# NIRVANALAN/LN3Diff

Hardware: NVIDIA H100
Metric: denoised-latents/sec (higher is better)
Workload: dtype bf16

## Files before the change

### ln3diff_b200/csrc/attention_wgmma.cu

```cuda
#include <cstdlib>

#include "common.cuh"
#include "ln3_internal.h"

namespace ln3 {

static constexpr int kQT = 128;
static constexpr int kKT = 128;
static constexpr int kHD = 64;
static constexpr int kTileBytes = 128 * kHD * 2;
static constexpr int kStages = 4;
static constexpr int kThreads = 2 * 128 + 32;
static constexpr int kFmhaSmem = 1024 + kTileBytes * (1 + 2 * kStages) + 256;

struct FmhaParams {
  int Lq, Lkv, Lkv2;
  int nb1, nb2;
  float scale_log2;
  int causal;
  __nv_bfloat16* out;
  long long o_ld, o_bs;
};

__global__ void __launch_bounds__(kThreads, 1)
fmha_fwd_kernel(const __grid_constant__ CUtensorMap tmap_q, const __grid_constant__ CUtensorMap tmap_k,
                const __grid_constant__ CUtensorMap tmap_v, const __grid_constant__ CUtensorMap tmap_k2,
                const __grid_constant__ CUtensorMap tmap_v2, const FmhaParams p) {
  extern __shared__ uint8_t smem_raw[];
  uint8_t* smem = reinterpret_cast<uint8_t*>((reinterpret_cast<uintptr_t>(smem_raw) + 1023) &
                                             ~static_cast<uintptr_t>(1023));
  uint8_t* sQ = smem;
  uint8_t* sK = sQ + kTileBytes;
  uint8_t* sV = sK + kStages * kTileBytes;
  uint64_t* bars = reinterpret_cast<uint64_t*>(sV + kStages * kTileBytes);
  uint64_t* q_full = bars;
  uint64_t* kv_full = bars + 1;
  uint64_t* kv_empty = bars + 1 + kStages;

  const int warp = threadIdx.x >> 5;
  const int lane = threadIdx.x & 31;
  const int q0 = blockIdx.x * kQT;
  const int h = blockIdx.y, b = blockIdx.z;
  const int nb1 = p.causal ? min(p.nb1, (min(q0 + kQT, p.Lq) - 1) / kKT + 1) : p.nb1;
  const int nblocks = nb1 + p.nb2;

  if (threadIdx.x == 0) {
    tma_prefetch_desc(&tmap_q);
    tma_prefetch_desc(&tmap_k);
    tma_prefetch_desc(&tmap_v);
    mbar_init(q_full, 1);
    for (int i = 0; i < kStages; ++i) {
      mbar_init(&kv_full[i], 1);
      mbar_init(&kv_empty[i], 2);
    }
    fence_barrier_init();
  }
  __syncthreads();
  pdl_launch_dependents();
  pdl_wait();

  if (warp == 8) {
    if (lane == 0) {
      mbar_arrive_expect_tx(q_full, kTileBytes);
      tma_load_3d(sQ, &tmap_q, q_full, h * kHD, q0, b);
      int stage = 0;
      uint32_t phase = 0;
      for (int j = 0; j < nblocks; ++j) {
        mbar_wait(&kv_empty[stage], phase ^ 1);
        mbar_arrive_expect_tx(&kv_full[stage], 2 * kTileBytes);
        const bool second = j >= nb1;
        const int row = (second ? j - nb1 : j) * kKT;
        tma_load_3d(sK + stage * kTileBytes, second ? &tmap_k2 : &tmap_k, &kv_full[stage], h * kHD, row, b);
        tma_load_3d(sV + stage * kTileBytes, second ? &tmap_v2 : &tmap_v, &kv_full[stage], h * kHD, row, b);
        if (++stage == kStages) {
          stage = 0;
          phase ^= 1;
        }
      }
    }
    return;
  }

  const int wg = warp >> 2;
  const int g = lane >> 2, q = lane & 3;
  const int r0 = q0 + wg * 64 + (warp & 3) * 16 + g;
  const uint64_t q_desc = make_smem_desc_sw128(smem_u32(sQ + wg * (64 * 128)), 16, 1024);
  const uint64_t k_desc0 = make_smem_desc_sw128(smem_u32(sK), 16, 1024);
  const uint64_t v_desc0 = make_smem_desc_sw128(smem_u32(sV), 16, 1024);

  float o[kHD / 2];
#pragma unroll
  for (int i = 0; i < kHD / 2; ++i) o[i] = 0.f;
  float m_run[2] = {-INFINITY, -INFINITY}, l_run[2] = {0.f, 0.f};
  mbar_wait(q_full, 0);

  int stage = 0;
  uint32_t phase = 0;
  for (int j = 0; j < nblocks; ++j) {
    const bool second = j >= nb1;
    const int kbase = (second ? j - nb1 : j) * kKT;
    const int klen = second ? p.Lkv2 : p.Lkv;
    mbar_wait(&kv_full[stage], phase);
    float s[kKT / 2];
    wgmma_fence();
#pragma unroll
    for (int k = 0; k < kHD / 16; ++k)
      wgmma_m64n128k16_ss(s, q_desc + 2 * k, k_desc0 + static_cast<uint32_t>(stage) * (kTileBytes >> 4) + 2 * k,
                          k != 0 ? 1u : 0u);
    wgmma_commit();
    wgmma_wait<0>();
#pragma unroll
    for (int i = 0; i < kKT / 2; ++i) reg_fence(s[i]);

    const bool need_mask = kbase + kKT > klen || (p.causal && !second && kbase + kKT - 1 > r0);
    float mx[2] = {-INFINITY, -INFINITY};
#pragma unroll
    for (int i = 0; i < kKT / 8; ++i) {
#pragma unroll
      for (int e = 0; e < 4; ++e) {
        float v = s[4 * i + e] * p.scale_log2;
        if (need_mask) {
          const int key = kbase + 8 * i + 2 * q + (e & 1);
          const int row = r0 + 8 * (e >> 1);
          if (key >= klen || (p.causal && !second && key > row)) v = -INFINITY;
        }
        s[4 * i + e] = v;
        mx[e >> 1] = fmaxf(mx[e >> 1], v);
      }
    }
    float alpha[2], m_use[2];
#pragma unroll
    for (int r = 0; r < 2; ++r) {
      mx[r] = fmaxf(mx[r], __shfl_xor_sync(0xffffffffu, mx[r], 1));
      mx[r] = fmaxf(mx[r], __shfl_xor_sync(0xffffffffu, mx[r], 2));
      const float m_new = fmaxf(m_run[r], mx[r]);
      m_use[r] = m_new == -INFINITY ? 0.f : m_new;
      alpha[r] = fast_exp2(m_run[r] - m_use[r]);
      m_run[r] = m_new;
      l_run[r] *= alpha[r];
    }
    uint32_t pa[kKT / 16][4];
#pragma unroll
    for (int kk = 0; kk < kKT / 16; ++kk) {
      float e[8];
#pragma unroll
      for (int t = 0; t < 8; ++t) {
        e[t] = fast_exp2(s[8 * kk + t] - m_use[(t >> 1) & 1]);
        l_run[(t >> 1) & 1] += e[t];
      }
      pa[kk][0] = pack_bf16x2(e[0], e[1]);
      pa[kk][1] = pack_bf16x2(e[2], e[3]);
      pa[kk][2] = pack_bf16x2(e[4], e[5]);
      pa[kk][3] = pack_bf16x2(e[6], e[7]);
    }
#pragma unroll
    for (int i = 0; i < kHD / 8; ++i) {
      o[4 * i] *= alpha[0]; o[4 * i + 1] *= alpha[0];
      o[4 * i + 2] *= alpha[1]; o[4 * i + 3] *= alpha[1];
    }
    wgmma_fence();
#pragma unroll
    for (int kk = 0; kk < kKT / 16; ++kk)
      wgmma_m64n64k16_rs_tb(o, pa[kk], v_desc0 + static_cast<uint32_t>(stage) * (kTileBytes >> 4) + kk * 128, 1u);
    wgmma_commit();
    wgmma_wait<0>();
#pragma unroll
    for (int i = 0; i < kHD / 2; ++i) reg_fence(o[i]);
    if ((threadIdx.x & 127) == 0) mbar_arrive(&kv_empty[stage]);
    if (++stage == kStages) {
      stage = 0;
      phase ^= 1;
    }
  }

#pragma unroll
  for (int r = 0; r < 2; ++r) {
    l_run[r] += __shfl_xor_sync(0xffffffffu, l_run[r], 1);
    l_run[r] += __shfl_xor_sync(0xffffffffu, l_run[r], 2);
  }
  const float inv[2] = {l_run[0] > 0.f ? 1.f / l_run[0] : 0.f, l_run[1] > 0.f ? 1.f / l_run[1] : 0.f};
#pragma unroll
  for (int r = 0; r < 2; ++r) {
    const int row = r0 + 8 * r;
    if (row >= p.Lq) continue;
    __nv_bfloat16* dst = p.out + b * p.o_bs + row * p.o_ld + h * kHD + 2 * q;
#pragma unroll
    for (int i = 0; i < kHD / 8; ++i)
      *reinterpret_cast<uint32_t*>(dst + 8 * i) = pack_bf16x2(o[4 * i + 2 * r] * inv[r], o[4 * i + 2 * r + 1] * inv[r]);
  }
}

int fmha_fwd(const ln3_fmha_args* a, cudaStream_t stream) {
  if (a->head_dim != kHD) return set_error(LN3_EUNSUPPORTED, "fmha: head_dim must be 64");
  if (a->B <= 0 || a->H <= 0 || a->Lq <= 0 || a->Lkv <= 0)
    return set_error(LN3_EINVAL, "fmha: empty problem");
  if ((a->q_ld | a->k_ld | a->v_ld | a->o_ld | a->q_bs | a->k_bs | a->v_bs | a->o_bs) % 8)
    return set_error(LN3_EINVAL, "fmha: strides must be multiples of 8 elements");
  if ((reinterpret_cast<uintptr_t>(a->q) | reinterpret_cast<uintptr_t>(a->k) |
       reinterpret_cast<uintptr_t>(a->v) | reinterpret_cast<uintptr_t>(a->out)) & 15)
    return set_error(LN3_EINVAL, "fmha: pointers must be 16-byte aligned");
  if (a->causal && (a->k2 != nullptr || a->v2 != nullptr))
    return set_error(LN3_EINVAL, "fmha: causal attention takes a single K/V source");
  const bool two = a->k2 != nullptr || a->v2 != nullptr;
  if (two) {
    if (!a->k2 || !a->v2 || a->Lkv2 <= 0) return set_error(LN3_EINVAL, "fmha: k2/v2/Lkv2 must be given together");
    if ((a->k2_ld | a->v2_ld | a->k2_bs | a->v2_bs) % 8 ||
        ((reinterpret_cast<uintptr_t>(a->k2) | reinterpret_cast<uintptr_t>(a->v2)) & 15))
      return set_error(LN3_EINVAL, "fmha: k2/v2 alignment");
  }
  if (a->B > 65535 || a->H > 65535) return set_error(LN3_EUNSUPPORTED, "fmha: batch or head count above 65535");
  static DeviceOnce once;
  if (int rc = once.run([] {
        cudaError_t e = cudaFuncSetAttribute(fmha_fwd_kernel, cudaFuncAttributeMaxDynamicSharedMemorySize, kFmhaSmem);
        return e == cudaSuccess ? LN3_OK : set_error(LN3_ECUDA, "fmha: cudaFuncSetAttribute: %s", cudaGetErrorString(e));
      }))
    return rc;
  CUtensorMap tq, tk, tv, tk2, tv2;
  int rc;
  const long long cols = static_cast<long long>(a->H) * kHD;
  if ((rc = make_tmap_3d_bf16(&tq, a->q, cols, a->Lq, a->B, a->q_ld, a->q_bs, kHD, kQT))) return rc;
  if ((rc = make_tmap_3d_bf16(&tk, a->k, cols, a->Lkv, a->B, a->k_ld, a->k_bs, kHD, kKT))) return rc;
  if ((rc = make_tmap_3d_bf16(&tv, a->v, cols, a->Lkv, a->B, a->v_ld, a->v_bs, kHD, kKT))) return rc;
  if (two) {
    if ((rc = make_tmap_3d_bf16(&tk2, a->k2, cols, a->Lkv2, a->B, a->k2_ld, a->k2_bs, kHD, kKT))) return rc;
    if ((rc = make_tmap_3d_bf16(&tv2, a->v2, cols, a->Lkv2, a->B, a->v2_ld, a->v2_bs, kHD, kKT))) return rc;
  } else {
    tk2 = tk;
    tv2 = tv;
  }
  FmhaParams p;
  p.Lq = a->Lq;
  p.Lkv = a->Lkv;
  p.Lkv2 = two ? a->Lkv2 : 0;
  p.nb1 = (a->Lkv + kKT - 1) / kKT;
  p.nb2 = two ? (a->Lkv2 + kKT - 1) / kKT : 0;
  p.scale_log2 = a->scale * 1.4426950408889634f;
  p.causal = a->causal ? 1 : 0;
  p.out = reinterpret_cast<__nv_bfloat16*>(a->out);
  p.o_ld = a->o_ld;
  p.o_bs = a->o_bs;
  const dim3 grid((a->Lq + kQT - 1) / kQT, a->H, a->B);
  cudaError_t e = launch_pdl(fmha_fwd_kernel, grid, dim3(kThreads), kFmhaSmem, stream, tq, tk, tv, tk2, tv2, p);
  if (e != cudaSuccess) return set_error(LN3_ECUDA, "fmha launch: %s", cudaGetErrorString(e));
  count_launch();
  return LN3_OK;
}

}
```

Before: 1.206.

## Make FMHA persistent with intra-warpgroup QK/PV overlap and warpgroup ping-pong

Turns the attention kernel into a persistent kernel with one CTA per SM looping over (q-tile, head, batch) work items. The Q buffer is now recycled through a new q_empty barrier. Within each warpgroup, the S=QK^T wgmma for the next block is issued together with the P·V wgmma for the current block, so softmax runs while the tensor cores work. Named barriers alternate the two consumer warpgroups' wgmma issue (ping-pong). This adds scheduling complexity and barrier ordering risk, and static round-robin tile assignment may load-balance poorly under causal masking.

```diff
diff --git a/ln3diff_b200/csrc/attention_wgmma.cu b/ln3diff_b200/csrc/attention_wgmma.cu
--- a/ln3diff_b200/csrc/attention_wgmma.cu
+++ b/ln3diff_b200/csrc/attention_wgmma.cu
@@ -11,16 +11,99 @@
 static constexpr int kTileBytes = 128 * kHD * 2;
 static constexpr int kStages = 4;
 static constexpr int kThreads = 2 * 128 + 32;
+static constexpr int kOrderBar = 1;
 static constexpr int kFmhaSmem = 1024 + kTileBytes * (1 + 2 * kStages) + 256;
 
 struct FmhaParams {
   int Lq, Lkv, Lkv2;
   int nb1, nb2;
+  int H, n_qt;
+  long long n_tiles;
   float scale_log2;
   int causal;
   __nv_bfloat16* out;
   long long o_ld, o_bs;
 };
+
+struct Tile {
+  int q0, h, b, nb1, nblocks;
+};
+
+__device__ __forceinline__ Tile decode_tile(const FmhaParams& p, long long t) {
+  Tile d;
+  const long long bh = t / p.n_qt;
+  d.q0 = static_cast<int>(t - bh * p.n_qt) * kQT;
+  d.h = static_cast<int>(bh % p.H);
+  d.b = static_cast<int>(bh / p.H);
+  d.nb1 = p.causal ? min(p.nb1, (min(d.q0 + kQT, p.Lq) - 1) / kKT + 1) : p.nb1;
+  d.nblocks = d.nb1 + p.nb2;
+  return d;
+}
+
+__device__ __forceinline__ void softmax_block(const FmhaParams& p, float* s, float* m_run, float* l_run,
+                                              float* alpha, int j, int nb1, int r0, int q) {
+  const bool second = j >= nb1;
+  const int kbase = (second ? j - nb1 : j) * kKT;
+  const int klen = second ? p.Lkv2 : p.Lkv;
+  const bool need_mask = kbase + kKT > klen || (p.causal && !second && kbase + kKT - 1 > r0);
+  float mx[2] = {-INFINITY, -INFINITY};
+#pragma unroll
+  for (int i = 0; i < kKT / 8; ++i) {
+#pragma unroll
+    for (int e = 0; e < 4; ++e) {
+      float v = __fmul_rn(s[4 * i + e], p.scale_log2);
+      if (need_mask) {
+        const int key = kbase + 8 * i + 2 * q + (e & 1);
+        const int row = r0 + 8 * (e >> 1);
+        if (key >= klen || (p.causal && !second && key > row)) v = -INFINITY;
+      }
+      s[4 * i + e] = v;
+      mx[e >> 1] = fmaxf(mx[e >> 1], v);
+    }
+  }
+  float m_use[2];
+#pragma unroll
+  for (int r = 0; r < 2; ++r) {
+    mx[r] = fmaxf(mx[r], __shfl_xor_sync(0xffffffffu, mx[r], 1));
+    mx[r] = fmaxf(mx[r], __shfl_xor_sync(0xffffffffu, mx[r], 2));
+    const float m_new = fmaxf(m_run[r], mx[r]);
+    m_use[r] = m_new == -INFINITY ? 0.f : m_new;
+    alpha[r] = fast_exp2(__fsub_rn(m_run[r], m_use[r]));
+    m_run[r] = m_new;
+  }
+#pragma unroll
+  for (int kk = 0; kk < kKT / 16; ++kk) {
+#pragma unroll
+    for (int t = 0; t < 8; ++t) {
+      const int r = (t >> 1) & 1;
+      const float e = fast_exp2(__fsub_rn(s[8 * kk + t], m_use[r]));
+      s[8 * kk + t] = e;
+      l_run[r] = (kk == 0 && (t == 0 || t == 2)) ? __fmaf_rn(alpha[r], l_run[r], e) : __fadd_rn(l_run[r], e);
+    }
+  }
+}
+
+__device__ __forceinline__ void pack_p(const float* s, uint32_t (*pa)[4]) {
+#pragma unroll
+  for (int kk = 0; kk < kKT / 16; ++kk) {
+    pa[kk][0] = pack_bf16x2(s[8 * kk + 0], s[8 * kk + 1]);
+    pa[kk][1] = pack_bf16x2(s[8 * kk + 2], s[8 * kk + 3]);
+    pa[kk][2] = pack_bf16x2(s[8 * kk + 4], s[8 * kk + 5]);
+    pa[kk][3] = pack_bf16x2(s[8 * kk + 6], s[8 * kk + 7]);
+  }
+}
+
+__device__ __forceinline__ void issue_s(float* s, uint64_t q_desc, uint64_t k_desc) {
+#pragma unroll
+  for (int k = 0; k < kHD / 16; ++k) wgmma_m64n128k16_ss(s, q_desc + 2 * k, k_desc + 2 * k, k != 0 ? 1u : 0u);
+  wgmma_commit();
+}
+
+__device__ __forceinline__ void issue_pv(float* o, const uint32_t (*pa)[4], uint64_t v_desc) {
+#pragma unroll
+  for (int kk = 0; kk < kKT / 16; ++kk) wgmma_m64n64k16_rs_tb(o, pa[kk], v_desc + kk * 128, 1u);
+  wgmma_commit();
+}
 
 __global__ void __launch_bounds__(kThreads, 1)
 fmha_fwd_kernel(const __grid_constant__ CUtensorMap tmap_q, const __grid_constant__ CUtensorMap tmap_k,
@@ -34,21 +117,19 @@
   uint8_t* sV = sK + kStages * kTileBytes;
   uint64_t* bars = reinterpret_cast<uint64_t*>(sV + kStages * kTileBytes);
   uint64_t* q_full = bars;
-  uint64_t* kv_full = bars + 1;
-  uint64_t* kv_empty = bars + 1 + kStages;
+  uint64_t* q_empty = bars + 1;
+  uint64_t* kv_full = bars + 2;
+  uint64_t* kv_empty = bars + 2 + kStages;
 
   const int warp = threadIdx.x >> 5;
   const int lane = threadIdx.x & 31;
-  const int q0 = blockIdx.x * kQT;
-  const int h = blockIdx.y, b = blockIdx.z;
-  const int nb1 = p.causal ? min(p.nb1, (min(q0 + kQT, p.Lq) - 1) / kKT + 1) : p.nb1;
-  const int nblocks = nb1 + p.nb2;
 
   if (threadIdx.x == 0) {
     tma_prefetch_desc(&tmap_q);
     tma_prefetch_desc(&tmap_k);
     tma_prefetch_desc(&tmap_v);
     mbar_init(q_full, 1);
+    mbar_init(q_empty, 2);
     for (int i = 0; i < kStages; ++i) {
       mbar_init(&kv_full[i], 1);
       mbar_init(&kv_empty[i], 2);
@@ -61,20 +142,24 @@
 
   if (warp == 8) {
     if (lane == 0) {
-      mbar_arrive_expect_tx(q_full, kTileBytes);
-      tma_load_3d(sQ, &tmap_q, q_full, h * kHD, q0, b);
       int stage = 0;
-      uint32_t phase = 0;
-      for (int j = 0; j < nblocks; ++j) {
-        mbar_wait(&kv_empty[stage], phase ^ 1);
-        mbar_arrive_expect_tx(&kv_full[stage], 2 * kTileBytes);
-        const bool second = j >= nb1;
-        const int row = (second ? j - nb1 : j) * kKT;
-        tma_load_3d(sK + stage * kTileBytes, second ? &tmap_k2 : &tmap_k, &kv_full[stage], h * kHD, row, b);
-        tma_load_3d(sV + stage * kTileBytes, second ? &tmap_v2 : &tmap_v, &kv_full[stage], h * kHD, row, b);
-        if (++stage == kStages) {
-          stage = 0;
-          phase ^= 1;
+      uint32_t phase = 0, tcount = 0;
+      for (long long t = blockIdx.x; t < p.n_tiles; t += gridDim.x, ++tcount) {
+        const Tile d = decode_tile(p, t);
+        mbar_wait_silent(q_empty, (tcount & 1) ^ 1);
+        mbar_arrive_expect_tx(q_full, kTileBytes);
+        tma_load_3d(sQ, &tmap_q, q_full, d.h * kHD, d.q0, d.b);
+        for (int j = 0; j < d.nblocks; ++j) {
+          mbar_wait_silent(&kv_empty[stage], phase ^ 1);
+          mbar_arrive_expect_tx(&kv_full[stage], 2 * kTileBytes);
+          const bool second = j >= d.nb1;
+          const int row = (second ? j - d.nb1 : j) * kKT;
+          tma_load_3d(sK + stage * kTileBytes, second ? &tmap_k2 : &tmap_k, &kv_full[stage], d.h * kHD, row, d.b);
+          tma_load_3d(sV + stage * kTileBytes, second ? &tmap_v2 : &tmap_v, &kv_full[stage], d.h * kHD, row, d.b);
+          if (++stage == kStages) {
+            stage = 0;
+            phase ^= 1;
+          }
         }
       }
     }
@@ -83,110 +168,104 @@
 
   const int wg = warp >> 2;
   const int g = lane >> 2, q = lane & 3;
-  const int r0 = q0 + wg * 64 + (warp & 3) * 16 + g;
+  const bool leader = (threadIdx.x & 127) == 0;
   const uint64_t q_desc = make_smem_desc_sw128(smem_u32(sQ + wg * (64 * 128)), 16, 1024);
   const uint64_t k_desc0 = make_smem_desc_sw128(smem_u32(sK), 16, 1024);
   const uint64_t v_desc0 = make_smem_desc_sw128(smem_u32(sV), 16, 1024);
 
-  float o[kHD / 2];
-#pragma unroll
-  for (int i = 0; i < kHD / 2; ++i) o[i] = 0.f;
-  float m_run[2] = {-INFINITY, -INFINITY}, l_run[2] = {0.f, 0.f};
-  mbar_wait(q_full, 0);
+  bool first_batch = true;
+  auto batch_begin = [&]() {
+    if (wg == 1 || !first_batch) named_bar_sync(kOrderBar + wg, 256);
+    first_batch = false;
+  };
+  auto batch_end = [&](bool last) {
+    if (wg == 0 || !last) named_bar_arrive(kOrderBar + (wg ^ 1), 256);
+  };
 
   int stage = 0;
-  uint32_t phase = 0;
-  for (int j = 0; j < nblocks; ++j) {
-    const bool second = j >= nb1;
-    const int kbase = (second ? j - nb1 : j) * kKT;
-    const int klen = second ? p.Lkv2 : p.Lkv;
-    mbar_wait(&kv_full[stage], phase);
+  uint32_t phase = 0, tcount = 0;
+  for (long long t = blockIdx.x; t < p.n_tiles; t += gridDim.x, ++tcount) {
+    const Tile d = decode_tile(p, t);
+    const bool last_tile = t + gridDim.x >= p.n_tiles;
+    const int r0 = d.q0 + wg * 64 + (warp & 3) * 16 + g;
+    float o[kHD / 2];
+#pragma unroll
+    for (int i = 0; i < kHD / 2; ++i) o[i] = 0.f;
+    float m_run[2] = {-INFINITY, -INFINITY}, l_run[2] = {0.f, 0.f}, alpha[2];
     float s[kKT / 2];
+    uint32_t pa[kKT / 16][4];
+
+    mbar_wait_silent(q_full, tcount & 1);
+    mbar_wait_silent(&kv_full[stage], phase);
+    batch_begin();
     wgmma_fence();
-#pragma unroll
-    for (int k = 0; k < kHD / 16; ++k)
-      wgmma_m64n128k16_ss(s, q_desc + 2 * k, k_desc0 + static_cast<uint32_t>(stage) * (kTileBytes >> 4) + 2 * k,
-                          k != 0 ? 1u : 0u);
-    wgmma_commit();
+    issue_s(s, q_desc, k_desc0 + static_cast<uint32_t>(stage) * (kTileBytes >> 4));
+    batch_end(false);
     wgmma_wait<0>();
 #pragma unroll
     for (int i = 0; i < kKT / 2; ++i) reg_fence(s[i]);
-
-    const bool need_mask = kbase + kKT > klen || (p.causal && !second && kbase + kKT - 1 > r0);
-    float mx[2] = {-INFINITY, -INFINITY};
-#pragma unroll
-    for (int i = 0; i < kKT / 8; ++i) {
-#pragma unroll
-      for (int e = 0; e < 4; ++e) {
-        float v = s[4 * i + e] * p.scale_log2;
-        if (need_mask) {
-          const int key = kbase + 8 * i + 2 * q + (e & 1);
-          const int row = r0 + 8 * (e >> 1);
-          if (key >= klen || (p.causal && !second && key > row)) v = -INFINITY;
-        }
-        s[4 * i + e] = v;
-        mx[e >> 1] = fmaxf(mx[e >> 1], v);
+    if (d.nblocks == 1 && leader) mbar_arrive(q_empty);
+    softmax_block(p, s, m_run, l_run, alpha, 0, d.nb1, r0, q);
+    pack_p(s, pa);
+
+    for (int j = 0; j + 1 < d.nblocks; ++j) {
+      const int cur = stage;
+      if (++stage == kStages) {
+        stage = 0;
+        phase ^= 1;
       }
-    }
-    float alpha[2], m_use[2];
-#pragma unroll
-    for (int r = 0; r < 2; ++r) {
-      mx[r] = fmaxf(mx[r], __shfl_xor_sync(0xffffffffu, mx[r], 1));
-      mx[r] = fmaxf(mx[r], __shfl_xor_sync(0xffffffffu, mx[r], 2));
-      const float m_new = fmaxf(m_run[r], mx[r]);
-      m_use[r] = m_new == -INFINITY ? 0.f : m_new;
-      alpha[r] = fast_exp2(m_run[r] - m_use[r]);
-      m_run[r] = m_new;
-      l_run[r] *= alpha[r];
-    }
-    uint32_t pa[kKT / 16][4];
-#pragma unroll
-    for (int kk = 0; kk < kKT / 16; ++kk) {
-      float e[8];
-#pragma unroll
-      for (int t = 0; t < 8; ++t) {
-        e[t] = fast_exp2(s[8 * kk + t] - m_use[(t >> 1) & 1]);
-        l_run[(t >> 1) & 1] += e[t];
+      mbar_wait_silent(&kv_full[stage], phase);
+      batch_begin();
+      wgmma_fence();
+      issue_s(s, q_desc, k_desc0 + static_cast<uint32_t>(stage) * (kTileBytes >> 4));
+      issue_pv(o, pa, v_desc0 + static_cast<uint32_t>(cur) * (kTileBytes >> 4));
+      batch_end(false);
+      wgmma_wait<1>();
+#pragma unroll
+      for (int i = 0; i < kKT / 2; ++i) reg_fence(s[i]);
+      if (j + 2 == d.nblocks && leader) mbar_arrive(q_empty);
+      softmax_block(p, s, m_run, l_run, alpha, j + 1, d.nb1, r0, q);
+      wgmma_wait<0>();
+#pragma unroll
+      for (int i = 0; i < kHD / 2; ++i) reg_fence(o[i]);
+      if (leader) mbar_arrive(&kv_empty[cur]);
+#pragma unroll
+      for (int i = 0; i < kHD / 8; ++i) {
+        o[4 * i] *= alpha[0]; o[4 * i + 1] *= alpha[0];
+        o[4 * i + 2] *= alpha[1]; o[4 * i + 3] *= alpha[1];
       }
-      pa[kk][0] = pack_bf16x2(e[0], e[1]);
-      pa[kk][1] = pack_bf16x2(e[2], e[3]);
-      pa[kk][2] = pack_bf16x2(e[4], e[5]);
-      pa[kk][3] = pack_bf16x2(e[6], e[7]);
-    }
-#pragma unroll
-    for (int i = 0; i < kHD / 8; ++i) {
-      o[4 * i] *= alpha[0]; o[4 * i + 1] *= alpha[0];
-      o[4 * i + 2] *= alpha[1]; o[4 * i + 3] *= alpha[1];
-    }
+      pack_p(s, pa);
+    }
+
+    batch_begin();
     wgmma_fence();
-#pragma unroll
-    for (int kk = 0; kk < kKT / 16; ++kk)
-      wgmma_m64n64k16_rs_tb(o, pa[kk], v_desc0 + static_cast<uint32_t>(stage) * (kTileBytes >> 4) + kk * 128, 1u);
-    wgmma_commit();
+    issue_pv(o, pa, v_desc0 + static_cast<uint32_t>(stage) * (kTileBytes >> 4));
+    batch_end(last_tile);
     wgmma_wait<0>();
 #pragma unroll
     for (int i = 0; i < kHD / 2; ++i) reg_fence(o[i]);
-    if ((threadIdx.x & 127) == 0) mbar_arrive(&kv_empty[stage]);
+    if (leader) mbar_arrive(&kv_empty[stage]);
     if (++stage == kStages) {
       stage = 0;
       phase ^= 1;
     }
-  }
-
-#pragma unroll
-  for (int r = 0; r < 2; ++r) {
-    l_run[r] += __shfl_xor_sync(0xffffffffu, l_run[r], 1);
-    l_run[r] += __shfl_xor_sync(0xffffffffu, l_run[r], 2);
-  }
-  const float inv[2] = {l_run[0] > 0.f ? 1.f / l_run[0] : 0.f, l_run[1] > 0.f ? 1.f / l_run[1] : 0.f};
-#pragma unroll
-  for (int r = 0; r < 2; ++r) {
-    const int row = r0 + 8 * r;
-    if (row >= p.Lq) continue;
-    __nv_bfloat16* dst = p.out + b * p.o_bs + row * p.o_ld + h * kHD + 2 * q;
-#pragma unroll
-    for (int i = 0; i < kHD / 8; ++i)
-      *reinterpret_cast<uint32_t*>(dst + 8 * i) = pack_bf16x2(o[4 * i + 2 * r] * inv[r], o[4 * i + 2 * r + 1] * inv[r]);
+
+#pragma unroll
+    for (int r = 0; r < 2; ++r) {
+      l_run[r] += __shfl_xor_sync(0xffffffffu, l_run[r], 1);
+      l_run[r] += __shfl_xor_sync(0xffffffffu, l_run[r], 2);
+    }
+    const float inv[2] = {l_run[0] > 0.f ? 1.f / l_run[0] : 0.f, l_run[1] > 0.f ? 1.f / l_run[1] : 0.f};
+#pragma unroll
+    for (int r = 0; r < 2; ++r) {
+      const int row = r0 + 8 * r;
+      if (row >= p.Lq) continue;
+      __nv_bfloat16* dst = p.out + d.b * p.o_bs + row * p.o_ld + d.h * kHD + 2 * q;
+#pragma unroll
+      for (int i = 0; i < kHD / 8; ++i)
+        *reinterpret_cast<uint32_t*>(dst + 8 * i) =
+            pack_bf16x2(o[4 * i + 2 * r] * inv[r], o[4 * i + 2 * r + 1] * inv[r]);
+    }
   }
 }
 
@@ -234,13 +313,17 @@
   p.Lkv2 = two ? a->Lkv2 : 0;
   p.nb1 = (a->Lkv + kKT - 1) / kKT;
   p.nb2 = two ? (a->Lkv2 + kKT - 1) / kKT : 0;
+  p.H = a->H;
+  p.n_qt = (a->Lq + kQT - 1) / kQT;
+  p.n_tiles = static_cast<long long>(p.n_qt) * a->H * a->B;
   p.scale_log2 = a->scale * 1.4426950408889634f;
   p.causal = a->causal ? 1 : 0;
   p.out = reinterpret_cast<__nv_bfloat16*>(a->out);
   p.o_ld = a->o_ld;
   p.o_bs = a->o_bs;
-  const dim3 grid((a->Lq + kQT - 1) / kQT, a->H, a->B);
-  cudaError_t e = launch_pdl(fmha_fwd_kernel, grid, dim3(kThreads), kFmhaSmem, stream, tq, tk, tv, tk2, tv2, p);
+  const int sms = device_sm_count();
+  const int grid = p.n_tiles < sms ? static_cast<int>(p.n_tiles) : sms;
+  cudaError_t e = launch_pdl(fmha_fwd_kernel, dim3(grid), dim3(kThreads), kFmhaSmem, stream, tq, tk, tv, tk2, tv2, p);
   if (e != cudaSuccess) return set_error(LN3_ECUDA, "fmha launch: %s", cudaGetErrorString(e));
   count_launch();
   return LN3_OK;
```

Measured after the change: 1.263, median of 6. 1.05x the previous value.
